# imkaywu/MVSKit

Hardware: AMD Instinct MI355X
Metric: patches/s (propagate+optim iteration), 12-view 1080p (higher is better)
Workload: dtype f32

## Files before the change

### include/mvskit_engine.h

```cpp
#ifndef MVSKIT_ENGINE_H
#define MVSKIT_ENGINE_H

#include <stddef.h>
#include <stdint.h>

#ifdef __cplusplus
extern "C" {
#endif

#ifndef MVS_MAX_IMAGES
#define MVS_MAX_IMAGES 32
#endif
#define MVS_LIST_CAP 16

typedef enum mvs_status {
    MVS_OK = 0,
    MVS_ERR_ARG = -1,
    MVS_ERR_STATE = -2,
    MVS_ERR_HIP = -3,
    MVS_ERR_CAPACITY = -4,
    MVS_ERR_NO_DEVICE = -5
} mvs_status;

typedef struct mvs_patch {
// ... 141 lines not shown
    MVS_PROBE_REFINE = 2,
    MVS_PROBE_POSTPROCESS = 3,
    MVS_PROBE_COST = 4,
    MVS_PROBE_MATH = 5,
    MVS_PROBE_REFINE_X = 6
} mvs_probe_op;
int mvs_engine_probe(mvs_engine* e, int op, int64_t n, const mvs_patch* in_rec, const float* in_f,
                     mvs_patch* out_rec, float* out_f, int32_t* out_i);

typedef struct mvs_timing {
    float index_ms;
    float sweep_ms;
    float commit_ms;
    int32_t sweep_launches;
    float exchange_ms;
    int64_t exchange_bytes;
    int64_t check_retried_cells;
} mvs_timing;
int mvs_engine_last_timing(mvs_engine* e, mvs_timing* t);

#ifdef __cplusplus
}
#endif
#endif
```

### mvskit_amd/csrc/mvs_engine.cpp

```cpp
#include <hip/hip_runtime.h>
#include <dlfcn.h>
#include <rccl/rccl.h>

#include <algorithm>
#include <climits>
#include <cmath>
#include <cstdio>
#include <cstdlib>
#include <cstring>
#include <string>
#include <vector>

#include "mvskit_engine.h"
#include "mvs_kernels.h"
#include "mvs_types.h"

static_assert(sizeof(mvs_patch) == sizeof(DPatch), "mvs_patch and DPatch must be the same bytes");
static_assert((MVS_LISTCAP == 16 || MVS_LISTCAP == 32 || MVS_LISTCAP == 64) && MVS_LISTCAP <= MVS_MAXI && MVS_MAX_IMAGES == MVS_MAXI, "limits out of sync");

namespace {
thread_local std::string g_err;

#define HIPCHK(expr)                                                                                       \
    do {                                                                                                   \
// ... 32 lines not shown
    }
    void release() { if (p) (void)hipFree(p); p = nullptr; cap = 0; }
};

namespace misc {
constexpr int stage_counter = 0;
constexpr int fill_evals = 1;
constexpr int neighbor_retry = 4;
constexpr int sweep_retry = 5;
constexpr int geo_bad = 6;
constexpr int group_edges = 7;
constexpr int trim_parts = 8;
constexpr int trim_nparts = 256;
constexpr int sweep_cursors = (trim_parts + trim_nparts + 15) / 16 * 16;
constexpr int sweep_cursor_words = MVS_SWEEP_QUEUES * MVS_SWEEP_CURSOR_STRIDE * (int)sizeof(uint32_t) / (int)sizeof(unsigned long long);
constexpr int words = sweep_cursors + sweep_cursor_words;
}
namespace fstat {
constexpr int neighbor_parts = 0;
constexpr int neighbor_cycles = 4096;
constexpr int exact_evals = 4112;
constexpr int words = exact_evals + 2048;
}

struct Rccl {
    void* h = nullptr;
    ncclResult_t (*GetUniqueId)(ncclUniqueId*) = nullptr;
    ncclResult_t (*CommInitRank)(ncclComm_t*, int, ncclUniqueId, int) = nullptr;
    ncclResult_t (*CommDestroy)(ncclComm_t) = nullptr;
    ncclResult_t (*CommCount)(const ncclComm_t, int*) = nullptr;
    ncclResult_t (*CommUserRank)(const ncclComm_t, int*) = nullptr;
// ... 90 lines not shown
    DevBuf<int32_t> group_edges;
    DevBuf<int32_t> cnt_alive, vcnt_alive;
    DevBuf<unsigned long long> dpgrid, best;
    DevBuf<uint32_t> dirty;
    bool dirty_marked = false;
    DevBuf<float4> geo;
    DevBuf<uint8_t> geo_ref;
    bool geo_valid = false;
    bool lists_dense[2] = {false, false};
    DevBuf<DPatch> staging;
    DevBuf<int32_t> job_stage, job_nstage, job_cnt, job_base_scan, kill_cnt, kill_base;
    DevBuf<unsigned long long> misc;
    DevBuf<DCounters> counters;
    DevBuf<int32_t> error_flag;
    DevBuf<int32_t> big_tables, retry_jobs;
    int64_t retried_cells = 0;
    int64_t pass_retried = 0;
    SweepArgs sa{};
    bool staged = false;
    bool counted = false;
    int64_t n_new = 0, n_kill = 0;
    std::vector<int32_t> h_per_view;
    DevBuf<DPatch> tmp_rec_in, tmp_rec_out;
    DevBuf<float> tmp_f_in, tmp_f_out;
    DevBuf<int32_t> tmp_i;
    DevBuf<uint8_t> tmp_bytes;
    hipEvent_t ev[6] = {nullptr, nullptr, nullptr, nullptr, nullptr, nullptr};
    mvs_timing timing{};
    mvs_filter_stats fstats{};
    int64_t fstats_exchange_bytes = 0;
// ... 586 lines not shown
        size_t free_b = 0, total_b = 0;
        if (hipMemGetInfo(&free_b, &total_b) == hipSuccess && total_b > 0) {
            pool_cap = std::max<int64_t>(std::min<int64_t>(pool_cap, (int64_t)(total_b / 6 / sizeof(DPatch))), std::min<int64_t>(pool_cap, nc));
            const double per_patch = 2.5 * (double)sizeof(DPatch) + 17.0;
            const int64_t fit = (int64_t)(0.6 * (double)free_b / per_patch);
            if (fit < pool_cap) pool_cap = std::max<int64_t>(fit, std::min<int64_t>(pool_cap, nc / 4 + 1024));
        }
    }
    e->ids.headroom = e->key.headroom = e->id32.headroom = e->id32_raw.headroom = e->vid32.headroom = true;
    e->geo.headroom = e->geo_ref.headroom = true;
    if (e->pool.ensure(pool_cap) || e->pool_alt.ensure(pool_cap) || e->kill.ensure(pool_cap) || e->kill_cnt.ensure(pool_cap + 2) || e->kill_base.ensure(pool_cap + 2)) return MVS_ERR_HIP;
    HIPCHK(hipMemsetAsync(e->kill.p, 0, (size_t)pool_cap, st));
    int64_t njobs_max = 0;
    for (int v = 0; v < nviews; ++v) njobs_max += (int64_t)((e->hviews[v].gw + 1) / 2) * e->hviews[v].gh;
    const int maxstage = (e->prm.view_propagation ? 3 : 2) * e->prm.cap * e->prm.max_propag;
    if (e->job_stage.ensure(njobs_max * maxstage) || e->job_nstage.ensure(njobs_max + 2) || e->job_cnt.ensure(njobs_max + 2) ||
        e->job_base_scan.ensure(njobs_max + 2))
        return MVS_ERR_HIP;
    const int64_t scan_n = std::max<int64_t>(std::max<int64_t>(nc, pool_cap), njobs_max);
    if (e->scan_tmp.ensure(scan_n / 256 + 4096)) return MVS_ERR_HIP;
    if (e->big_tables.ensure((int64_t)256 * 16384) || e->retry_jobs.ensure(std::max<int64_t>(njobs_max, 16))) return MVS_ERR_HIP;
    if (e->uf_parent.ensure(pool_cap) || e->uf_size.ensure(pool_cap) || e->dirty.ensure((nc + 31) / 32 + 1) || e->fstat_buf.ensure(fstat::words)) return MVS_ERR_HIP;
    if (e->staging.ensure(std::max<int64_t>(pool_cap / 2, 1024))) return MVS_ERR_HIP;
    if (e->tmp_rec_out.ensure(16)) return MVS_ERR_HIP;
    HIPCHK(hipStreamSynchronize(st));
    e->pool_n = 0;
    e->have_views = true;
    e->staged = false;
    return MVS_OK;
}

int mvs_engine_grid_dims(mvs_engine* e, int view, int* gw, int* gh) {
// ... 286 lines not shown
    if (e->kill.p && e->pool_n > 0) (void)hipMemsetAsync(e->kill.p, 0, (size_t)e->pool_n, e->stream);
    (void)hipStreamSynchronize(e->stream);
    e->staged = false; e->counted = false;
}
static int pass_impl(mvs_engine* e, int iter, int pass, mvs_counters* out) {
    if (!e || !e->have_views) { g_err = "mvs_engine_pass: views not set"; return MVS_ERR_STATE; }
    if (e->staged) { g_err = "mvs_engine_pass: the previous pass was not committed"; return MVS_ERR_STATE; }
    HIPCHK(hipSetDevice(e->cfg.device));
    hipStream_t st = e->stream;
    HIPCHK(hipEventRecord(e->ev[0], st));
    unsigned long long trimmed = 0;
    {
        Range rg("mvs:index");
        if (int r = build_index(e, &trimmed)) return r;
    }
    HIPCHK(hipEventRecord(e->ev[1], st));
    Range rg_sweep(pass & 1 ? "mvs:sweep colour 1" : "mvs:sweep colour 0");
    SweepArgs& a = e->sa;
    memset(&a, 0, sizeof a);
    a.iter = iter; a.inc = (iter % 2 == 0) ? 1 : -1; a.colour = pass & 1;
    int64_t nj = 0;
    const bool ranged = e->cfg.shard_count > 1;
    for (int v = ranged ? 0 : e->cfg.view_begin; v < e->cfg.nviews; v += ranged ? 1 : e->cfg.view_stride) {
        a.sweep_views[a.nsweep_views] = v;
        a.job_base[a.nsweep_views] = (int32_t)nj;
        ++a.nsweep_views;
        nj += (int64_t)((e->hviews[v].gw + 1) / 2) * e->hviews[v].gh;
    }
    a.njobs = nj;
    a.job_lo = 0; a.job_hi = nj;
    if (ranged) {
        const int split_mode = getenv("MVS_SPLIT_PROXY") ? atoi(getenv("MVS_SPLIT_PROXY")) : 2;
// ... 10 lines not shown
            HIPCHK(hipMemsetAsync(e->tmp_i.p, 0xff, (size_t)(N + 1) * sizeof(int32_t), st));
            mvsk_job_cuts(e->job_base_scan.p, nj, N, e->tmp_i.p, st);
            int32_t tw = 0;
            HIPCHK(hipMemcpyAsync(cuts.data(), e->tmp_i.p, (size_t)(N + 1) * sizeof(int32_t), hipMemcpyDeviceToHost, st));
            HIPCHK(hipMemcpyAsync(&tw, e->job_base_scan.p + nj, sizeof tw, hipMemcpyDeviceToHost, st));
            HIPCHK(hipStreamSynchronize(st));
            total_work = tw;
        }
        cuts[0] = 0; cuts[N] = (int32_t)nj;
        for (int r = 1; r < N; ++r) {
            if (total_work <= 0 || cuts[r] < 0) cuts[r] = (int32_t)(nj * r / N);
            cuts[r] = std::max(cuts[r], cuts[r - 1]);
        }
        a.job_lo = cuts[R];
        a.job_hi = cuts[R + 1];
        HIPCHK(hipMemsetAsync(e->job_nstage.p, 0, (size_t)nj * sizeof(int32_t), st));
    }
    a.staging = e->staging.p; a.staging_cap = e->staging.cap;
    a.stage_counter = e->misc.p + misc::stage_counter;
    a.job_stage = e->job_stage.p; a.job_nstage = e->job_nstage.p;
    a.maxstage = (e->prm.view_propagation ? 3 : 2) * e->prm.cap * e->prm.max_propag;
    a.kill = e->kill.p;
    a.counters = e->counters.p;
    a.error_flag = e->error_flag.p;
    if (want_vgrid(e)) {
        if (int r = e->big_tables.ensure((int64_t)256 * 16384)) return r;
        if (int r = e->retry_jobs.ensure(std::max<int64_t>(nj, 16))) return r;
    }
    a.big_tables = e->big_tables.p; a.retry_jobs = e->retry_jobs.p; a.nretry = reinterpret_cast<int32_t*>(e->misc.p + misc::sweep_retry);
    HIPCHK(hipMemsetAsync(e->misc.p + misc::sweep_retry, 0, sizeof(unsigned long long), st));
    HIPCHK(hipMemsetAsync(e->misc.p + misc::stage_counter, 0, sizeof(unsigned long long), st));
    a.cursors = reinterpret_cast<uint32_t*>(e->misc.p + misc::sweep_cursors);
    HIPCHK(hipMemsetAsync(e->misc.p + misc::sweep_cursors, 0, misc::sweep_cursor_words * sizeof(unsigned long long), st));
    HIPCHK(hipMemsetAsync(e->counters.p, 0, MVS_COUNTER_SLOTS * sizeof(DCounters), st));
    HIPCHK(hipMemsetAsync(e->error_flag.p, 0, sizeof(int32_t), st));
    const DParams p = current_params(e);
    const RefineSel rs = refine_sel(e);
    mvsk_sweep(p, a, rs, st);
    e->pass_retried = 0;
    if (want_vgrid(e)) {
        int32_t nretry = 0;
        HIPCHK(hipMemcpyAsync(&nretry, a.nretry, sizeof nretry, hipMemcpyDeviceToHost, st));
        HIPCHK(hipStreamSynchronize(st));
        e->pass_retried = nretry;
        if (nretry > 0) { mvsk_sweep_retry(p, a, nretry, rs, st); e->retried_cells += nretry; }
    }
    HIPCHK(hipEventRecord(e->ev[2], st));
    std::vector<DCounters> hcs(MVS_COUNTER_SLOTS);
    int32_t herr = 0;
    unsigned long long fill[2] = {0, 0};
    HIPCHK(hipMemcpyAsync(fill, e->misc.p + misc::fill_evals, sizeof fill, hipMemcpyDeviceToHost, st));
    HIPCHK(hipMemcpyAsync(hcs.data(), e->counters.p, hcs.size() * sizeof(DCounters), hipMemcpyDeviceToHost, st));
    HIPCHK(hipMemcpyAsync(&herr, e->error_flag.p, sizeof herr, hipMemcpyDeviceToHost, st));
    HIPCHK(hipStreamSynchronize(st));
    HIPCHK(hipGetLastError());
    mvs_counters sum{};
    for (const DCounters& c : hcs) add_counters(sum, c);
    sum.evals += fill[0]; sum.view_evals += fill[1]; sum.trimmed = (int64_t)trimmed;
    float ms = 0.0f;
    (void)hipEventElapsedTime(&ms, e->ev[0], e->ev[1]); e->timing.index_ms = ms;
    (void)hipEventElapsedTime(&ms, e->ev[1], e->ev[2]); e->timing.sweep_ms = ms;
    e->timing.commit_ms = 0.0f; e->timing.sweep_launches = 1; e->timing.exchange_ms = 0.0f; e->timing.exchange_bytes = 0;
    e->timing.check_retried_cells = e->pass_retried;
    e->staged = true; e->counted = false;
    if (out) *out = sum;
#ifdef MVS_STAGE_TIMING
    {
        unsigned long long stage[16] = {0};
        for (const DCounters& c : hcs)
            for (int k = 0; k < 16; ++k) stage[k] = (k == 12 || k == 13) ? std::max(stage[k], c.stage[k]) : stage[k] + c.stage[k];
        static const char* nm[8] = {"wave", "generate", "pre", "refine", "post", "check", "stage", "prologue"};
        fprintf(stderr, "[stage cycles]");
        for (int k = 0; k < 8; ++k) fprintf(stderr, " %s %.1f%%", nm[k], 100.0 * (double)stage[k] / (double)(stage[0] ? stage[0] : 1));
        static const char* nm2[4] = {"gain", "search", "sort", "quad"};
        for (int k = 0; k < 4; ++k) fprintf(stderr, " %s %.1f%%", nm2[k], 100.0 * (double)stage[8 + k] / (double)(stage[0] ? stage[0] : 1));
        fprintf(stderr, " setRefImage pairs %.1f%% choice %.1f%%", 100.0 * (double)stage[14] / (double)(stage[0] ? stage[0] : 1), 100.0 * (double)stage[15] / (double)(stage[0] ? stage[0] : 1));
        fprintf(stderr, "  (wave cycles %.3e; max visited %llu, max neighbours %llu)\n", (double)stage[0], stage[12], stage[13]);
    }
#endif
#ifdef MVS_FAULT_INJECTION
// ... 214 lines not shown
    memset(&total, 0, sizeof total);
    mvs_timing tt{};
    for (int pass = 0; pass < 2; ++pass) {
        mvs_counters c;
        memset(&c, 0, sizeof c);
        const int rp = mvs_engine_pass(e, iter, pass, &c);
        if (e && e->comm) {
            if (int r = mvs_engine_exchange(e)) return r;
        } else {
            if (rp) { if (e && e->staged) { const std::string keep = g_err; discard_pass(e); g_err = keep; } return rp; }
            if (int r = mvs_engine_commit_local(e)) return r;
        }
        add_counters(total, c);
        tt.index_ms += e->timing.index_ms; tt.sweep_ms += e->timing.sweep_ms; tt.commit_ms += e->timing.commit_ms; tt.sweep_launches += 1;
        tt.exchange_ms += e->timing.exchange_ms; tt.exchange_bytes += e->timing.exchange_bytes; tt.check_retried_cells += e->timing.check_retried_cells;
    }
    e->timing = tt;
    if (out) *out = total;
    return MVS_OK;
}

int mvs_engine_filter(mvs_engine* e, int64_t* removed4) {
    if (!e || !e->have_views) { g_err = "mvs_engine_filter: views not set"; return MVS_ERR_STATE; }
    if (e->staged) { g_err = "mvs_engine_filter: a pass is waiting for its commit"; return MVS_ERR_STATE; }
    HIPCHK(hipSetDevice(e->cfg.device));
    hipStream_t st = e->stream;
    int64_t rem[4] = {0, 0, 0, 0};
    Range rg("mvs:Filter::run");
    FilterRun fr{e};
    if (fr.multi()) { if (int r = e->comm_counts.ensure(MVS_XCHG_WORDS * (1 + (int64_t)e->comm_world))) return r; }
// ... 212 lines not shown
```

### mvskit_amd/csrc/mvs_kernels.h

```cpp
#pragma once
#include <hip/hip_runtime.h>
#include "mvs_types.h"

void mvsk_rgb_to_rgba(const uint8_t* rgb, uint32_t* out, int64_t n, hipStream_t st);
void mvsk_rgba_to_rgb(const uint32_t* in, uint8_t* rgb, int64_t n, hipStream_t st);
void mvsk_pyr_down(const uint32_t* src, int pw, int ph, uint32_t* dst, int w, int h, hipStream_t st);
void mvsk_mask_down(const uint8_t* src, int pw, int ph, uint8_t* dst, int w, int h, hipStream_t st);
void mvsk_mask_binarise(uint8_t* m, int64_t n, hipStream_t st);
void mvsk_exclusive_scan(const int32_t* in, int32_t* out, int64_t n, int32_t* tmp, hipStream_t st);
void mvsk_index_count(const DParams& prm, int32_t* cnt, int32_t* vcnt, unsigned long long* total, hipStream_t st);
void mvsk_exclusive_scan_off(const int32_t* in, csr_off_t* out, int64_t n, csr_off_t* tmp, hipStream_t st);
void mvsk_index_fill(const DParams& prm, int vgrid, const csr_off_t* start, int32_t* cursor, unsigned long long* ids, hipStream_t st);
void mvsk_index_fill_direct(const DParams& prm, int vgrid, const csr_off_t* start, int32_t* cursor, int32_t* id32, hipStream_t st);
void mvsk_index_sort_trim(const DParams& prm, const csr_off_t* start, unsigned long long* ids, int do_trim, unsigned long long* trimmed, hipStream_t st);
void mvsk_index_finalize(const DParams& prm, int vgrid, const csr_off_t* start, unsigned long long* ids, int32_t* id32, int32_t* cnt_alive, hipStream_t st);
void mvsk_index_pack(const DParams& prm, const csr_off_t* start, const csr_off_t* start2, const int32_t* cnt_alive, const unsigned long long* ids, const int32_t* id32_in,
                     ListKey* key, int32_t* id32_out, hipStream_t st);
void mvsk_depth_maps(const DParams& prm, unsigned long long* dp, const uint32_t* dirty, hipStream_t st);
void mvsk_depth_mark_dirty(const DParams& prm, const uint8_t* kill, unsigned long long* dp, uint32_t* dirty, hipStream_t st);
void mvsk_best_ncc_map(const DParams& prm, int view, unsigned long long* best, hipStream_t st);
void mvsk_map_extract(const DParams& prm, int view, int kind, const unsigned long long* sel, float* depth, float* normal, int32_t* ids, int ncells, hipStream_t st);
void mvsk_fill_ncc(const DParams& prm, unsigned long long* evals, hipStream_t st);
struct RefineSel { int simplex; int max_evals; float xtol; };
size_t mvsk_sweep_lds_bytes(const DParams& prm);
void mvsk_sweep(const DParams& prm, const SweepArgs& a, const RefineSel& rs, hipStream_t st);
void mvsk_sweep_retry(const DParams& prm, const SweepArgs& a, int nretry, const RefineSel& rs, hipStream_t st);
void mvsk_job_work(const DParams& prm, const SweepArgs& a, int mode, int shift, int32_t* work, hipStream_t st);
void mvsk_job_cuts(const int32_t* scan, int64_t njobs, int n, int32_t* cuts, hipStream_t st);
void mvsk_commit_count(const SweepArgs& a, int32_t* cnt, hipStream_t st);
void mvsk_commit_copy(const SweepArgs& a, const int32_t* base, DPatch* dst, int64_t dst_cap, int32_t* per_view, int keep_key, hipStream_t st);
void mvsk_kill_count(const uint8_t* kill, int64_t n, int32_t* cnt, hipStream_t st);
void mvsk_kill_export(const uint8_t* kill, int64_t n, const int32_t* base, int32_t* ids, int64_t cap, hipStream_t st);
void mvsk_apply_kill_flags(DPatch* pool, uint8_t* kill, int64_t n, hipStream_t st);
void mvsk_apply_kill_ids(DPatch* pool, const int32_t* ids, int64_t n, int64_t pool_n, hipStream_t st);
void mvsk_append_records(DPatch* pool, int64_t pool_n, const DPatch* recs, int64_t n, hipStream_t st);
void mvsk_alive_count(const DPatch* pool, int64_t n, int32_t* cnt, hipStream_t st);
void mvsk_alive_gather(const DPatch* pool, int64_t n, const int32_t* base, DPatch* out, int64_t cap, hipStream_t st);
void mvsk_filter_vimages(const DParams& prm, int additive, int64_t first, int64_t last, const uint32_t* dirty, hipStream_t st);
void mvsk_geo_pack(const DPatch* pool, int64_t n, float4* geo, uint8_t* ref, int* bad, hipStream_t st);
void mvsk_filter_outside(const DParams& prm, uint8_t* kill, int64_t first, int64_t last, hipStream_t st);
void mvsk_filter_exact(const DParams& prm, uint8_t* kill, unsigned long long* evals, unsigned long long* stage, int64_t first, int64_t last, hipStream_t st);
void mvsk_filter_neighbor(const DParams& prm, uint8_t* kill, int32_t* retry, int32_t* nretry, int32_t* overflow, unsigned long long* stats, int64_t first, int64_t last, hipStream_t st);
// ... 21 lines not shown
```

### mvskit_amd/csrc/mvs_kernels.hip

```cpp
#include <hip/hip_runtime.h>
#include <algorithm>
#include "mvs_device.cuh"
#include "mvs_check.cuh"
#include "mvs_kernels.h"

using namespace mvsdev;

__global__ void k_rgb_to_rgba(const uint8_t* __restrict__ rgb, uint32_t* __restrict__ out, int64_t n) {
    const int64_t i = (int64_t)blockIdx.x * blockDim.x + threadIdx.x;
    if (i >= n) return;
    const uint8_t* p = rgb + 3 * i;
    out[i] = (uint32_t)p[0] | ((uint32_t)p[1] << 8) | ((uint32_t)p[2] << 16);
}
__global__ void k_rgba_to_rgb(const uint32_t* __restrict__ in, uint8_t* __restrict__ rgb, int64_t n) {
    const int64_t i = (int64_t)blockIdx.x * blockDim.x + threadIdx.x;
    if (i >= n) return;
    const uint32_t t = in[i];
    rgb[3 * i] = t & 255u; rgb[3 * i + 1] = (t >> 8) & 255u; rgb[3 * i + 2] = (t >> 16) & 255u;
}
__global__ void k_pyr_down(const uint32_t* __restrict__ src, int pw, int ph, uint32_t* __restrict__ dst, int w, int h) {
    const int x = blockIdx.x * blockDim.x + threadIdx.x, y = blockIdx.y * blockDim.y + threadIdx.y;
    if (x >= w || y >= h) return;
    const float base[4] = {1.0f, 3.0f, 3.0f, 1.0f};
    float c0 = 0.0f, c1 = 0.0f, c2 = 0.0f;
// ... 293 lines not shown
        if (wc.lane == 0) p->ncc = ncc;
    }
    if (wc.lane == 0 && wc.evals) { atomicAdd(evals, (unsigned long long)wc.evals); atomicAdd(evals + 1, (unsigned long long)wc.view_evals); }
}

DEV bool rank_before(float na, int a, float nb, int b) { return (na != nb) ? (na > nb) : (a < b); }
DEV void job_cell(const DParams& prm, const SweepArgs& a, int64_t job, int& v, int& cx, int& cy) {
    int s = 0;
    while (s + 1 < a.nsweep_views && job >= a.job_base[s + 1]) ++s;
    v = a.sweep_views[s];
    const int gw = (prm.views + v)->gw, halfw = (gw + 1) / 2;
    const int local = (int)(job - a.job_base[s]);
    cy = local / halfw;
    cx = 2 * (local % halfw) + ((a.colour + cy) & 1);
}
DEV bool job_has_source(const DParams& prm, const SweepArgs& a, int64_t job) {
    int v, cx, cy;
    job_cell(prm, a, job, v, cx, cy);
    const DView* vw = prm.views + v;
    const int gw = vw->gw, gh = vw->gh;
    if (cx >= gw || cy >= gh) return false;
    const int sxs[2] = {cx, cx - a.inc}, sys[2] = {cy - a.inc, cy};
    bool has = false;
    for (int k = 0; k < 2; ++k) {
        if (sxs[k] < 0 || gw <= sxs[k] || sys[k] < 0 || gh <= sys[k]) continue;
        const int g = vw->cell_base + sys[k] * gw + sxs[k];
        has |= prm.csr_cnt[g] > 0;
    }
    if (prm.view_propagation) has |= prm.csr_cnt[vw->cell_base + cy * gw + cx] > 0;
    return has;
}
__global__ void k_job_work(DParams prm, SweepArgs a, int mode, int shift, int32_t* __restrict__ work) {
    const int64_t job = (int64_t)blockIdx.x * blockDim.x + threadIdx.x;
    if (job >= a.njobs) return;
    int v, cx, cy;
    job_cell(prm, a, job, v, cx, cy);
    const DView* vw = prm.views + v;
    const int gw = vw->gw, gh = vw->gh;
    int w = 0;
    if (cx < gw && cy < gh) {
        const int sxs[3] = {cx, cx - a.inc, cx}, sys[3] = {cy - a.inc, cy, cy};
        const int nsrc = prm.view_propagation ? 3 : 2;
        int n = 0;
        for (int k = 0; k < nsrc; ++k) {
            if (sxs[k] < 0 || gw <= sxs[k] || sys[k] < 0 || gh <= sys[k]) continue;
            const int g = vw->cell_base + sys[k] * gw + sxs[k];
            const csr_off_t sb = prm.csr_start[g];
            const int sn = prm.csr_cnt[g];
            for (int j = 0; j < sn; ++j) n += ((pgrid_ref(prm, sb + j) == v) != (k == 2)) ? 1 : 0;
        }
        if (mode == 1) w = n;
        else {
            const int trials = n * prm.max_propag;
            const int room = max(prm.cap - prm.csr_cnt[vw->cell_base + cy * gw + cx], 0);
            const int full = min(trials, (room * 5 + 3) / 4);
            w = 32 * full + 2 * (trials - full);
        }
    }
    work[job] = (w + (1 << shift) - 1) >> shift;
}
__global__ void k_job_cuts(const int32_t* __restrict__ scan, int64_t njobs, int n, int32_t* __restrict__ cuts) {
    const int64_t job = (int64_t)blockIdx.x * blockDim.x + threadIdx.x;
    if (job >= njobs) return;
    const long long total = scan[njobs], p0 = scan[job], p1 = scan[job + 1];
    if (p0 == p1) return;
    for (int r = 1; r < n; ++r) {
        const long long target = total * r / n;
        if (p0 <= target && target < p1) cuts[r] = (int32_t)job;
    }
}

#ifndef MVS_SWEEP_WAVES
#define MVS_SWEEP_WAVES 3
#endif
#ifdef MVS_STAGE_TIMING
#define ST_NOW() ((unsigned long long)__builtin_amdgcn_s_memtime())
#define ST_ADD(k, t0) { const unsigned long long t1_ = ST_NOW(); st_acc[k] += t1_ - (t0); (t0) = t1_; }
#else
#define ST_ADD(k, t0)
#endif
#ifndef MVS_XCD_CHUNK
#define MVS_XCD_CHUNK 128
#endif
struct SweepAcc {
    unsigned cand, pref, patch, f0, f1, ins, rep;
    unsigned long long evals, view_evals;
#ifdef MVS_STAGE_TIMING
    unsigned long long stage[16];
#endif
};
DEV SweepAcc sweep_acc_zero() {
    SweepAcc acc;
    acc.cand = acc.pref = acc.patch = acc.f0 = acc.f1 = acc.ins = acc.rep = 0u;
    acc.evals = acc.view_evals = 0ull;
#ifdef MVS_STAGE_TIMING
    for (int k = 0; k < 16; ++k) acc.stage[k] = 0ull;
#endif
// ... 157 lines not shown
        return;
    }
    if (wc.lane == 0) a.job_nstage[job] = ns;
    {
        acc->cand += n_cand; acc->pref += n_pref; acc->patch += n_patch; acc->f0 += n_f0; acc->f1 += n_f1; acc->ins += n_ins; acc->rep += n_rep;
        acc->evals += wc.evals; acc->view_evals += wc.view_evals;
#ifdef MVS_STAGE_TIMING
        st_acc[0] = ST_NOW() - st_begin;
        for (int k = 0; k < 12; ++k) acc->stage[k] += st_acc[k];
        acc->stage[12] = max(acc->stage[12], st_acc[12]); acc->stage[13] = max(acc->stage[13], st_acc[13]);
        acc->stage[14] += wc.st_acc[3]; acc->stage[15] += wc.st_acc[4];
#endif
    }
}

#ifndef MVS_SWEEP_TAKE
#define MVS_SWEEP_TAKE 1
#endif
static_assert(MVS_SWEEP_TAKE <= 64 && MVS_XCD_CHUNK % MVS_SWEEP_TAKE == 0, "a take is a part of one chunk, a lane per job");
template <bool SIMPLEX>
DEV void sweep_resident(const DParams& prm, const SweepArgs& a, int* s_scratch, float* s_texs, int max_evals, float xtol) {
    WaveCtx wc = make_wave_ctx(prm);
    SweepAcc acc = sweep_acc_zero();
    const int nchunks = (int)((a.job_hi - a.job_lo + MVS_XCD_CHUNK - 1) / MVS_XCD_CHUNK);
    constexpr unsigned per = MVS_XCD_CHUNK / MVS_SWEEP_TAKE;
    for (unsigned step = 0; step < MVS_SWEEP_QUEUES; ++step) {
        const unsigned q = (blockIdx.x + step) & (MVS_SWEEP_QUEUES - 1u);
        const unsigned ntake = (unsigned)((nchunks - (int)q + MVS_SWEEP_QUEUES - 1) / MVS_SWEEP_QUEUES) * per;
        for (;;) {
            unsigned k = 0;
            if (wc.lane == 0) k = atomicAdd(a.cursors + q * MVS_SWEEP_CURSOR_STRIDE, 1u);
            k = (unsigned)rfl((int)k);
            if (k >= ntake) break;
            const int64_t base = a.job_lo + ((int64_t)q + (int64_t)MVS_SWEEP_QUEUES * (k / per)) * MVS_XCD_CHUNK + (int64_t)(k % per) * MVS_SWEEP_TAKE;
            const int64_t mine = base + wc.lane;
            bool has = false;
            if (wc.lane < MVS_SWEEP_TAKE && mine < a.job_hi) {
                a.job_nstage[mine] = 0;
                has = job_has_source(prm, a, mine);
            }
            unsigned long long t = ballot(has);
            while (t) {
                const int l = __ffsll((long long)t) - 1;
                t &= t - 1ull;
                __syncthreads();
                sweep_cell<false, SIMPLEX>(prm, a, wc, &acc, base + l, s_scratch, s_texs, nullptr, max_evals, xtol);
            }
        }
    }
    if (wc.lane == 0) sweep_acc_flush(a, acc, blockIdx.x & (MVS_COUNTER_SLOTS - 1));
}
__global__ __launch_bounds__(64, MVS_SWEEP_WAVES) void k_sweep(DParams prm, SweepArgs a) {
    __shared__ int s_scratch[192];
    extern __shared__ float s_texs[];
    sweep_resident<false>(prm, a, s_scratch, s_texs, 0, 0.0f);
}
__global__ __launch_bounds__(64, MVS_SWEEP_WAVES) void k_sweep_simplex(DParams prm, SweepArgs a, int max_evals, float xtol) {
    __shared__ int s_scratch[192];
    extern __shared__ float s_texs[];
    sweep_resident<true>(prm, a, s_scratch, s_texs, max_evals, xtol);
}
template <bool SIMPLEX>
// ... 576 lines not shown
    const size_t texs = MVS_FRAME1_LDS_BYTES + (ln * 3 * prm.wsz + ln * (ln - 1) / 2) * sizeof(float);
#endif
    const size_t chk = (size_t)MVS_CHECK_LDS_FLOATS * sizeof(float);
    const size_t need = texs > chk ? texs : chk;
    return need > (size_t)MVS_FRAME_LDS_BYTES ? need : (size_t)MVS_FRAME_LDS_BYTES;
}
void mvsk_sweep(const DParams& prm, const SweepArgs& a, const RefineSel& rs, hipStream_t st) {
    const int64_t nloc = a.job_hi - a.job_lo;
    if (nloc <= 0) return;
    static const size_t pad = getenv("MVS_SWEEP_LDS_PAD") ? (size_t)atol(getenv("MVS_SWEEP_LDS_PAD")) : 0;
    const size_t lds = mvsk_sweep_lds_bytes(prm) + pad;
    int dev = 0, cus = 0;
    (void)hipGetDevice(&dev);
    if (hipDeviceGetAttribute(&cus, hipDeviceAttributeMultiprocessorCount, dev) != hipSuccess || cus <= 0) { (void)hipGetLastError(); cus = 256; }
    int64_t nblocks = (int64_t)cus * 4 * MVS_SWEEP_WAVES;
    nblocks = std::min(nblocks, (nloc + MVS_SWEEP_TAKE - 1) / MVS_SWEEP_TAKE);
    if (const char* g = getenv("MVS_SWEEP_GRID")) {
        const long cap = atol(g);
        if (cap > 0) nblocks = std::min<int64_t>(nblocks, cap);
    }
    if (rs.simplex) hipLaunchKernelGGL(k_sweep_simplex, dim3((unsigned)nblocks), dim3(64), lds, st, prm, a, rs.max_evals, rs.xtol);
    else hipLaunchKernelGGL(k_sweep, dim3((unsigned)nblocks), dim3(64), lds, st, prm, a);
}
void mvsk_job_work(const DParams& prm, const SweepArgs& a, int mode, int shift, int32_t* work, hipStream_t st) {
    if (a.njobs > 0) hipLaunchKernelGGL(k_job_work, dim3(nblk(a.njobs, 256)), dim3(256), 0, st, prm, a, mode, shift, work);
}
void mvsk_job_cuts(const int32_t* scan, int64_t njobs, int n, int32_t* cuts, hipStream_t st) {
    if (njobs > 0) hipLaunchKernelGGL(k_job_cuts, dim3(nblk(njobs, 256)), dim3(256), 0, st, scan, njobs, n, cuts);
}
void mvsk_sweep_retry(const DParams& prm, const SweepArgs& a, int nretry, const RefineSel& rs, hipStream_t st) {
    if (nretry <= 0) return;
    const dim3 grid((unsigned)std::min(nretry, MVS_BIG_SLOTS));
    if (rs.simplex) hipLaunchKernelGGL(k_sweep_retry_simplex, grid, dim3(64), mvsk_sweep_lds_bytes(prm), st, prm, a, nretry, rs.max_evals, rs.xtol);
    else hipLaunchKernelGGL(k_sweep_retry, grid, dim3(64), mvsk_sweep_lds_bytes(prm), st, prm, a, nretry);
}
void mvsk_commit_count(const SweepArgs& a, int32_t* cnt, hipStream_t st) { hipLaunchKernelGGL(k_commit_count, dim3(nblk(a.njobs, 256)), dim3(256), 0, st, a, cnt); }
void mvsk_commit_copy(const SweepArgs& a, const int32_t* base, DPatch* dst, int64_t dst_cap, int32_t* per_view, int keep_key, hipStream_t st) {
    hipLaunchKernelGGL(k_commit_copy, dim3(nblk(a.njobs, 256)), dim3(256), 0, st, a, base, dst, dst_cap, per_view, keep_key);
}
void mvsk_kill_count(const uint8_t* kill, int64_t n, int32_t* cnt, hipStream_t st) { if (n > 0) hipLaunchKernelGGL(k_kill_count, dim3(nblk(n, 256)), dim3(256), 0, st, kill, n, cnt); }
// ... 89 lines not shown
```

### mvskit_amd/csrc/mvs_types.h

```cpp
#pragma once
#include <stdint.h>

#define MVS_WAVE 64
#define MVS_MAXLEV 7
#ifndef MVS_LISTCAP
#define MVS_LISTCAP 16
#endif
#if MVS_LISTCAP > 32
#define MVS_MAXI 64
#else
#define MVS_MAXI 32
#endif
#define MVS_MAXVIEWS 64
#define MVS_CAPMAX 32
#define MVS_NEWBASE 0x40000000

#define MVS_FLAG_ALIVE 1
#define MVS_FLAG_SETTLED 2
struct DPatch {
    float coord[4];
    float normal[4];
    float ncc, dscale, ascale, tmp;
    int32_t nimages, nvimages, flags, id;
    uint8_t images[MVS_MAXI];
// ... 70 lines not shown
    int64_t njobs;
    int64_t job_lo, job_hi;
    DPatch* staging;
    int64_t staging_cap;
    unsigned long long* stage_counter;
    int32_t* job_stage;
    int32_t* job_nstage;
    int32_t maxstage;
    uint8_t* kill;
    DCounters* counters;
    int32_t* error_flag;
    int32_t* big_tables;
    int32_t* retry_jobs;
    int32_t* nretry;
    uint32_t* cursors;
};
```

### mvskit_amd/engine.py

```python
from __future__ import annotations

import ctypes as C
import os

import numpy as np

from . import build
from . import synth
from .synth import MAX_IMAGES, PATCH_DTYPE

PROBE_NCC, PROBE_PREPROCESS, PROBE_REFINE, PROBE_POSTPROCESS, PROBE_COST, PROBE_MATH, PROBE_REFINE_X = range(7)
REFINE_HALVING, REFINE_CONVERGED = 0, 1

EXPORTS = [
    "mvs_last_error", "mvs_device_count", "mvs_default_config", "mvs_engine_create", "mvs_engine_destroy",
    "mvs_engine_set_views", "mvs_engine_grid_dims", "mvs_engine_get_pyramid", "mvs_engine_set_thresholds",
    "mvs_engine_get_thresholds", "mvs_engine_update_threshold", "mvs_engine_upload_patches",
    "mvs_engine_clear_patches", "mvs_engine_num_patches", "mvs_engine_download_patches", "mvs_engine_propagate",
    "mvs_engine_pass", "mvs_engine_export_counts", "mvs_engine_export_device", "mvs_engine_commit_device",
    "mvs_engine_commit_local", "mvs_engine_depth_normal_map", "mvs_engine_probe", "mvs_engine_last_timing",
    "mvs_engine_filter", "mvs_comm_unique_id", "mvs_engine_comm_init", "mvs_engine_comm_attach", "mvs_engine_comm_release",
    "mvs_engine_exchange", "mvs_list_cap", "mvs_engine_filter_stats", "mvs_patch_bytes", "mvs_engine_reserve", "mvs_engine_comm_info",
    "mvs_default_refiner", "mvs_engine_set_refiner", "mvs_engine_export_ply", "mvs_engine_seed_patches",
]
# ... 22 lines not shown

class SeedView(C.Structure):
    _fields_ = [("normals", C.c_void_p), ("mask", C.c_void_p)]


class Counters(C.Structure):
    _fields_ = [(n, C.c_int64) for n in ("candidates", "prefiltered", "patches", "fail0", "fail1", "inserted",
                                         "replaced", "evals", "view_evals", "trimmed")]

    def as_dict(self):
        return {n: int(getattr(self, n)) for n, _ in self._fields_}


class Timing(C.Structure):
    _fields_ = [("index_ms", C.c_float), ("sweep_ms", C.c_float), ("commit_ms", C.c_float), ("sweep_launches", C.c_int32),
                ("exchange_ms", C.c_float), ("exchange_bytes", C.c_int64), ("check_retried_cells", C.c_int64)]


class FilterStats(C.Structure):
    _fields_ = [(n, C.c_float) for n in ("outside_ms", "exact_ms", "neighbor_ms", "groups_ms", "rebuild_ms", "total_ms")] + \
               [(n, C.c_int64) for n in ("patches_in", "exact_patches", "exact_view_evals", "neighbor_patches", "neighbor_tasks", "neighbor_entries",
                                         "neighbor_visited", "neighbor_accepted", "neighbor_retried", "exchange_bytes")]


class EngineError(RuntimeError):

    def __init__(self, msg, status=None):
        super().__init__(msg)
        self.status = status


# ... 265 lines not shown
        r, w, cc, cr = C.c_int(), C.c_int(), C.c_int(), C.c_int()
        self.L.mvs_engine_comm_info.argtypes = [C.c_void_p] + [C.POINTER(C.c_int)] * 4
        self._check(self.L.mvs_engine_comm_info(self.h, C.byref(r), C.byref(w), C.byref(cc), C.byref(cr)))
        return {"rank": r.value, "world": w.value, "comm_count": cc.value, "comm_rank": cr.value}

    def comm_release(self):
        self._check(self.L.mvs_engine_comm_release(self.h))

    def exchange(self):
        self._check(self.L.mvs_engine_exchange(self.h))

    def timing(self):
        t = Timing()
        self._check(self.L.mvs_engine_last_timing(self.h, C.byref(t)))
        return {"index_ms": t.index_ms, "sweep_ms": t.sweep_ms, "commit_ms": t.commit_ms, "sweep_launches": t.sweep_launches,
                "exchange_ms": t.exchange_ms, "exchange_bytes": int(t.exchange_bytes), "check_retried_cells": int(t.check_retried_cells)}

    def depth_normal_map(self, view, kind):
        gw, gh = self.grid_dims(view)
        d = np.zeros((gh, gw), np.float32)
        n = np.zeros((gh, gw, 3), np.float32)
        ids = np.zeros((gh, gw), np.int32)
        self._check(self.L.mvs_engine_depth_normal_map(self.h, view, kind, _ptr(d), _ptr(n), _ptr(ids)))
        return d, n, ids

    def probe(self, op, recs=None, values=None):
        if op == PROBE_MATH:
            x = np.ascontiguousarray(values, dtype=np.float32)
            out = np.zeros((x.shape[0], 5), np.float32)
            self._check(self.L.mvs_engine_probe(self.h, op, x.shape[0], None, _ptr(x), None, _ptr(out), None))
            return out
# ... 8 lines not shown
```

Measured before the change: 28.90 million.

## Compact sweep jobs into per-queue lists before the resident sweep kernel

Adds a pre-pass that flags each job with at least one same-view trial source, scans the flags and scatters the surviving job ids into a compacted list with per-queue bounds. The resident sweep kernel then pulls jobs straight from this list instead of claiming 128-job chunks and ballot-checking each lane for a source. The source test is now stricter, counting matching-view entries rather than any non-empty neighbour cell, so fewer empty jobs should reach the heavy sweep. The cost is three extra launches plus a scan per pass, and the job_nstage reset moves into the list kernel.

```diff
diff --git a/include/mvskit_engine.h b/include/mvskit_engine.h
--- a/include/mvskit_engine.h
+++ b/include/mvskit_engine.h
@@ -179,6 +179,7 @@
     float commit_ms;
     int32_t sweep_launches;
     float exchange_ms;
+    int32_t sweep_jobs_listed;
     int64_t exchange_bytes;
     int64_t check_retried_cells;
 } mvs_timing;
diff --git a/mvskit_amd/csrc/mvs_engine.cpp b/mvskit_amd/csrc/mvs_engine.cpp
--- a/mvskit_amd/csrc/mvs_engine.cpp
+++ b/mvskit_amd/csrc/mvs_engine.cpp
@@ -70,7 +70,10 @@
 constexpr int trim_nparts = 256;
 constexpr int sweep_cursors = (trim_parts + trim_nparts + 15) / 16 * 16;
 constexpr int sweep_cursor_words = MVS_SWEEP_QUEUES * MVS_SWEEP_CURSOR_STRIDE * (int)sizeof(uint32_t) / (int)sizeof(unsigned long long);
-constexpr int words = sweep_cursors + sweep_cursor_words;
+constexpr int sweep_list_bounds = sweep_cursors + sweep_cursor_words;
+constexpr int sweep_list_bound_words = (MVS_SWEEP_QUEUES + 1 + 1) / 2;
+constexpr int words = sweep_list_bounds + sweep_list_bound_words;
+constexpr int64_t job_list_pad = 1024 + 2;
 }
 namespace fstat {
 constexpr int neighbor_parts = 0;
@@ -191,6 +194,7 @@
     DevBuf<DCounters> counters;
     DevBuf<int32_t> error_flag;
     DevBuf<int32_t> big_tables, retry_jobs;
+    DevBuf<int32_t> job_list;
     int64_t retried_cells = 0;
     int64_t pass_retried = 0;
     SweepArgs sa{};
@@ -807,8 +811,8 @@
     int64_t njobs_max = 0;
     for (int v = 0; v < nviews; ++v) njobs_max += (int64_t)((e->hviews[v].gw + 1) / 2) * e->hviews[v].gh;
     const int maxstage = (e->prm.view_propagation ? 3 : 2) * e->prm.cap * e->prm.max_propag;
-    if (e->job_stage.ensure(njobs_max * maxstage) || e->job_nstage.ensure(njobs_max + 2) || e->job_cnt.ensure(njobs_max + 2) ||
-        e->job_base_scan.ensure(njobs_max + 2))
+    if (e->job_stage.ensure(njobs_max * maxstage) || e->job_nstage.ensure(njobs_max + 2) || e->job_cnt.ensure(njobs_max + misc::job_list_pad) ||
+        e->job_base_scan.ensure(njobs_max + misc::job_list_pad) || e->job_list.ensure(std::max<int64_t>(njobs_max, 16)))
         return MVS_ERR_HIP;
     const int64_t scan_n = std::max<int64_t>(std::max<int64_t>(nc, pool_cap), njobs_max);
     if (e->scan_tmp.ensure(scan_n / 256 + 4096)) return MVS_ERR_HIP;
@@ -1125,8 +1129,6 @@
         Range rg("mvs:index");
         if (int r = build_index(e, &trimmed)) return r;
     }
-    HIPCHK(hipEventRecord(e->ev[1], st));
-    Range rg_sweep(pass & 1 ? "mvs:sweep colour 1" : "mvs:sweep colour 0");
     SweepArgs& a = e->sa;
     memset(&a, 0, sizeof a);
     a.iter = iter; a.inc = (iter % 2 == 0) ? 1 : -1; a.colour = pass & 1;
@@ -1167,7 +1169,6 @@
         }
         a.job_lo = cuts[R];
         a.job_hi = cuts[R + 1];
-        HIPCHK(hipMemsetAsync(e->job_nstage.p, 0, (size_t)nj * sizeof(int32_t), st));
     }
     a.staging = e->staging.p; a.staging_cap = e->staging.cap;
     a.stage_counter = e->misc.p + misc::stage_counter;
@@ -1184,11 +1185,18 @@
     HIPCHK(hipMemsetAsync(e->misc.p + misc::sweep_retry, 0, sizeof(unsigned long long), st));
     HIPCHK(hipMemsetAsync(e->misc.p + misc::stage_counter, 0, sizeof(unsigned long long), st));
     a.cursors = reinterpret_cast<uint32_t*>(e->misc.p + misc::sweep_cursors);
-    HIPCHK(hipMemsetAsync(e->misc.p + misc::sweep_cursors, 0, misc::sweep_cursor_words * sizeof(unsigned long long), st));
+    HIPCHK(hipMemsetAsync(e->misc.p + misc::sweep_cursors, 0, (misc::sweep_cursor_words + misc::sweep_list_bound_words) * sizeof(unsigned long long), st));
     HIPCHK(hipMemsetAsync(e->counters.p, 0, MVS_COUNTER_SLOTS * sizeof(DCounters), st));
     HIPCHK(hipMemsetAsync(e->error_flag.p, 0, sizeof(int32_t), st));
     const DParams p = current_params(e);
     const RefineSel rs = refine_sel(e);
+    if (int r = e->job_list.ensure(std::max<int64_t>(nj, 16))) return r;
+    if (e->job_cnt.ensure(nj + misc::job_list_pad) || e->job_base_scan.ensure(nj + misc::job_list_pad)) return MVS_ERR_HIP;
+    int32_t* list_bounds = reinterpret_cast<int32_t*>(e->misc.p + misc::sweep_list_bounds);
+    a.job_list = e->job_list.p; a.list_bounds = list_bounds;
+    mvsk_job_list(p, a, e->job_cnt.p, e->job_base_scan.p, reinterpret_cast<int32_t*>(e->scan_tmp.p), e->job_list.p, list_bounds, st);
+    HIPCHK(hipEventRecord(e->ev[1], st));
+    Range rg_sweep(pass & 1 ? "mvs:sweep colour 1" : "mvs:sweep colour 0");
     mvsk_sweep(p, a, rs, st);
     e->pass_retried = 0;
     if (want_vgrid(e)) {
@@ -1205,6 +1213,8 @@
     HIPCHK(hipMemcpyAsync(fill, e->misc.p + misc::fill_evals, sizeof fill, hipMemcpyDeviceToHost, st));
     HIPCHK(hipMemcpyAsync(hcs.data(), e->counters.p, hcs.size() * sizeof(DCounters), hipMemcpyDeviceToHost, st));
     HIPCHK(hipMemcpyAsync(&herr, e->error_flag.p, sizeof herr, hipMemcpyDeviceToHost, st));
+    int32_t hbounds[MVS_SWEEP_QUEUES + 1];
+    HIPCHK(hipMemcpyAsync(hbounds, list_bounds, sizeof hbounds, hipMemcpyDeviceToHost, st));
     HIPCHK(hipStreamSynchronize(st));
     HIPCHK(hipGetLastError());
     mvs_counters sum{};
@@ -1215,8 +1225,13 @@
     (void)hipEventElapsedTime(&ms, e->ev[1], e->ev[2]); e->timing.sweep_ms = ms;
     e->timing.commit_ms = 0.0f; e->timing.sweep_launches = 1; e->timing.exchange_ms = 0.0f; e->timing.exchange_bytes = 0;
     e->timing.check_retried_cells = e->pass_retried;
+    e->timing.sweep_jobs_listed = hbounds[MVS_SWEEP_QUEUES];
     e->staged = true; e->counted = false;
     if (out) *out = sum;
+#ifdef MVS_JOBLIST_COUNTS
+    fprintf(stderr, "[job list] iter %d colour %d: jobs %lld, with any source entry %llu, listed %llu\n", iter, pass & 1, (long long)(a.job_hi - a.job_lo),
+            hcs[0].stage[0], hcs[0].stage[1]);
+#endif
 #ifdef MVS_STAGE_TIMING
     {
         unsigned long long stage[16] = {0};
@@ -1461,6 +1476,7 @@
         add_counters(total, c);
         tt.index_ms += e->timing.index_ms; tt.sweep_ms += e->timing.sweep_ms; tt.commit_ms += e->timing.commit_ms; tt.sweep_launches += 1;
         tt.exchange_ms += e->timing.exchange_ms; tt.exchange_bytes += e->timing.exchange_bytes; tt.check_retried_cells += e->timing.check_retried_cells;
+        tt.sweep_jobs_listed += e->timing.sweep_jobs_listed;
     }
     e->timing = tt;
     if (out) *out = total;
diff --git a/mvskit_amd/csrc/mvs_kernels.h b/mvskit_amd/csrc/mvs_kernels.h
--- a/mvskit_amd/csrc/mvs_kernels.h
+++ b/mvskit_amd/csrc/mvs_kernels.h
@@ -26,6 +26,8 @@
 void mvsk_sweep(const DParams& prm, const SweepArgs& a, const RefineSel& rs, hipStream_t st);
 void mvsk_sweep_retry(const DParams& prm, const SweepArgs& a, int nretry, const RefineSel& rs, hipStream_t st);
 void mvsk_job_work(const DParams& prm, const SweepArgs& a, int mode, int shift, int32_t* work, hipStream_t st);
+int mvsk_job_list_seg(const SweepArgs& a);
+void mvsk_job_list(const DParams& prm, const SweepArgs& a, int32_t* flags, int32_t* scan, int32_t* scan_tmp, int32_t* list, int32_t* bounds, hipStream_t st);
 void mvsk_job_cuts(const int32_t* scan, int64_t njobs, int n, int32_t* cuts, hipStream_t st);
 void mvsk_commit_count(const SweepArgs& a, int32_t* cnt, hipStream_t st);
 void mvsk_commit_copy(const SweepArgs& a, const int32_t* base, DPatch* dst, int64_t dst_cap, int32_t* per_view, int keep_key, hipStream_t st);
diff --git a/mvskit_amd/csrc/mvs_kernels.hip b/mvskit_amd/csrc/mvs_kernels.hip
--- a/mvskit_amd/csrc/mvs_kernels.hip
+++ b/mvskit_amd/csrc/mvs_kernels.hip
@@ -331,45 +331,37 @@
     cy = local / halfw;
     cx = 2 * (local % halfw) + ((a.colour + cy) & 1);
 }
-DEV bool job_has_source(const DParams& prm, const SweepArgs& a, int64_t job) {
+DEV int job_trial_sources(const DParams& prm, const SweepArgs& a, int64_t job, int* dest) {
     int v, cx, cy;
     job_cell(prm, a, job, v, cx, cy);
     const DView* vw = prm.views + v;
     const int gw = vw->gw, gh = vw->gh;
-    if (cx >= gw || cy >= gh) return false;
-    const int sxs[2] = {cx, cx - a.inc}, sys[2] = {cy - a.inc, cy};
-    bool has = false;
-    for (int k = 0; k < 2; ++k) {
+    *dest = -1;
+    if (cx >= gw || cy >= gh) return 0;
+    *dest = vw->cell_base + cy * gw + cx;
+    const int sxs[3] = {cx, cx - a.inc, cx}, sys[3] = {cy - a.inc, cy, cy};
+    const int nsrc = prm.view_propagation ? 3 : 2;
+    int n = 0;
+    for (int k = 0; k < nsrc; ++k) {
         if (sxs[k] < 0 || gw <= sxs[k] || sys[k] < 0 || gh <= sys[k]) continue;
         const int g = vw->cell_base + sys[k] * gw + sxs[k];
-        has |= prm.csr_cnt[g] > 0;
-    }
-    if (prm.view_propagation) has |= prm.csr_cnt[vw->cell_base + cy * gw + cx] > 0;
-    return has;
+        const csr_off_t sb = prm.csr_start[g];
+        const int sn = min(prm.csr_cnt[g], MVS_CAPMAX);
+        for (int j = 0; j < sn; ++j) n += ((pgrid_ref(prm, sb + j) == v) != (k == 2)) ? 1 : 0;
+    }
+    return n;
 }
 __global__ void k_job_work(DParams prm, SweepArgs a, int mode, int shift, int32_t* __restrict__ work) {
     const int64_t job = (int64_t)blockIdx.x * blockDim.x + threadIdx.x;
     if (job >= a.njobs) return;
-    int v, cx, cy;
-    job_cell(prm, a, job, v, cx, cy);
-    const DView* vw = prm.views + v;
-    const int gw = vw->gw, gh = vw->gh;
+    int dest;
+    const int n = job_trial_sources(prm, a, job, &dest);
     int w = 0;
-    if (cx < gw && cy < gh) {
-        const int sxs[3] = {cx, cx - a.inc, cx}, sys[3] = {cy - a.inc, cy, cy};
-        const int nsrc = prm.view_propagation ? 3 : 2;
-        int n = 0;
-        for (int k = 0; k < nsrc; ++k) {
-            if (sxs[k] < 0 || gw <= sxs[k] || sys[k] < 0 || gh <= sys[k]) continue;
-            const int g = vw->cell_base + sys[k] * gw + sxs[k];
-            const csr_off_t sb = prm.csr_start[g];
-            const int sn = prm.csr_cnt[g];
-            for (int j = 0; j < sn; ++j) n += ((pgrid_ref(prm, sb + j) == v) != (k == 2)) ? 1 : 0;
-        }
+    if (dest >= 0) {
         if (mode == 1) w = n;
         else {
             const int trials = n * prm.max_propag;
-            const int room = max(prm.cap - prm.csr_cnt[vw->cell_base + cy * gw + cx], 0);
+            const int room = max(prm.cap - prm.csr_cnt[dest], 0);
             const int full = min(trials, (room * 5 + 3) / 4);
             w = 32 * full + 2 * (trials - full);
         }
@@ -387,6 +379,48 @@
     }
 }
 
+#ifndef MVS_XCD_CHUNK
+#define MVS_XCD_CHUNK 128
+#endif
+DEV int64_t list_slot_job(const SweepArgs& a, int64_t slot, int seg) {
+    const int64_t q = slot / seg, r = slot % seg;
+    return a.job_lo + ((r / MVS_XCD_CHUNK) * MVS_SWEEP_QUEUES + q) * MVS_XCD_CHUNK + r % MVS_XCD_CHUNK;
+}
+__global__ void k_job_list(DParams prm, SweepArgs a, int seg, int32_t* __restrict__ flags) {
+    const int64_t t = (int64_t)blockIdx.x * blockDim.x + threadIdx.x;
+    if (t < a.njobs) a.job_nstage[t] = 0;
+    if (t >= (int64_t)MVS_SWEEP_QUEUES * seg) return;
+    const int64_t job = list_slot_job(a, t, seg);
+    int dest = -1;
+    const int n = job < a.job_hi ? job_trial_sources(prm, a, job, &dest) : 0;
+    flags[t] = n > 0 ? 1 : 0;
+#ifdef MVS_JOBLIST_COUNTS
+    bool any = false;
+    if (dest >= 0) {
+        int v, cx, cy;
+        job_cell(prm, a, job, v, cx, cy);
+        const DView* vw = prm.views + v;
+        const int sxs[3] = {cx, cx - a.inc, cx}, sys[3] = {cy - a.inc, cy, cy};
+        for (int k = 0; k < (prm.view_propagation ? 3 : 2); ++k)
+            if (0 <= sxs[k] && sxs[k] < vw->gw && 0 <= sys[k] && sys[k] < vw->gh) any |= prm.csr_cnt[vw->cell_base + sys[k] * vw->gw + sxs[k]] > 0;
+    }
+    const unsigned long long m_any = __ballot(any), m_listed = __ballot(n > 0);
+    if ((threadIdx.x & 63) == 0) {
+        if (m_any) atomicAdd(&a.counters->stage[0], (unsigned long long)__popcll(m_any));
+        if (m_listed) atomicAdd(&a.counters->stage[1], (unsigned long long)__popcll(m_listed));
+    }
+#endif
+}
+__global__ void k_job_scatter(SweepArgs a, int seg, const int32_t* __restrict__ scan, int32_t* __restrict__ list, int32_t* __restrict__ bounds) {
+    const int64_t t = (int64_t)blockIdx.x * blockDim.x + threadIdx.x;
+    const int64_t nslots = (int64_t)MVS_SWEEP_QUEUES * seg;
+    if (t >= nslots) return;
+    const int32_t pos = scan[t];
+    if (t % seg == 0) bounds[t / seg] = pos;
+    if (t == nslots - 1) bounds[MVS_SWEEP_QUEUES] = scan[nslots];
+    if (scan[t + 1] != pos) list[pos] = (int32_t)list_slot_job(a, t, seg);
+}
+
 #ifndef MVS_SWEEP_WAVES
 #define MVS_SWEEP_WAVES 3
 #endif
@@ -395,9 +429,6 @@
 #define ST_ADD(k, t0) { const unsigned long long t1_ = ST_NOW(); st_acc[k] += t1_ - (t0); (t0) = t1_; }
 #else
 #define ST_ADD(k, t0)
-#endif
-#ifndef MVS_XCD_CHUNK
-#define MVS_XCD_CHUNK 128
 #endif
 struct SweepAcc {
     unsigned cand, pref, patch, f0, f1, ins, rep;
@@ -585,38 +616,23 @@
     }
 }
 
-#ifndef MVS_SWEEP_TAKE
-#define MVS_SWEEP_TAKE 1
-#endif
-static_assert(MVS_SWEEP_TAKE <= 64 && MVS_XCD_CHUNK % MVS_SWEEP_TAKE == 0, "a take is a part of one chunk, a lane per job");
 template <bool SIMPLEX>
 DEV void sweep_resident(const DParams& prm, const SweepArgs& a, int* s_scratch, float* s_texs, int max_evals, float xtol) {
     WaveCtx wc = make_wave_ctx(prm);
     SweepAcc acc = sweep_acc_zero();
-    const int nchunks = (int)((a.job_hi - a.job_lo + MVS_XCD_CHUNK - 1) / MVS_XCD_CHUNK);
-    constexpr unsigned per = MVS_XCD_CHUNK / MVS_SWEEP_TAKE;
     for (unsigned step = 0; step < MVS_SWEEP_QUEUES; ++step) {
         const unsigned q = (blockIdx.x + step) & (MVS_SWEEP_QUEUES - 1u);
-        const unsigned ntake = (unsigned)((nchunks - (int)q + MVS_SWEEP_QUEUES - 1) / MVS_SWEEP_QUEUES) * per;
+        const int32_t qbegin = a.list_bounds[q];
+        const unsigned ntake = (unsigned)(a.list_bounds[q + 1] - qbegin);
+        if (ntake == 0u) continue;
         for (;;) {
             unsigned k = 0;
             if (wc.lane == 0) k = atomicAdd(a.cursors + q * MVS_SWEEP_CURSOR_STRIDE, 1u);
             k = (unsigned)rfl((int)k);
             if (k >= ntake) break;
-            const int64_t base = a.job_lo + ((int64_t)q + (int64_t)MVS_SWEEP_QUEUES * (k / per)) * MVS_XCD_CHUNK + (int64_t)(k % per) * MVS_SWEEP_TAKE;
-            const int64_t mine = base + wc.lane;
-            bool has = false;
-            if (wc.lane < MVS_SWEEP_TAKE && mine < a.job_hi) {
-                a.job_nstage[mine] = 0;
-                has = job_has_source(prm, a, mine);
-            }
-            unsigned long long t = ballot(has);
-            while (t) {
-                const int l = __ffsll((long long)t) - 1;
-                t &= t - 1ull;
-                __syncthreads();
-                sweep_cell<false, SIMPLEX>(prm, a, wc, &acc, base + l, s_scratch, s_texs, nullptr, max_evals, xtol);
-            }
+            const int64_t job = a.job_list[qbegin + (int32_t)k];
+            __syncthreads();
+            sweep_cell<false, SIMPLEX>(prm, a, wc, &acc, job, s_scratch, s_texs, nullptr, max_evals, xtol);
         }
     }
     if (wc.lane == 0) sweep_acc_flush(a, acc, blockIdx.x & (MVS_COUNTER_SLOTS - 1));
@@ -1223,7 +1239,7 @@
     (void)hipGetDevice(&dev);
     if (hipDeviceGetAttribute(&cus, hipDeviceAttributeMultiprocessorCount, dev) != hipSuccess || cus <= 0) { (void)hipGetLastError(); cus = 256; }
     int64_t nblocks = (int64_t)cus * 4 * MVS_SWEEP_WAVES;
-    nblocks = std::min(nblocks, (nloc + MVS_SWEEP_TAKE - 1) / MVS_SWEEP_TAKE);
+    nblocks = std::min(nblocks, nloc);
     if (const char* g = getenv("MVS_SWEEP_GRID")) {
         const long cap = atol(g);
         if (cap > 0) nblocks = std::min<int64_t>(nblocks, cap);
@@ -1233,6 +1249,19 @@
 }
 void mvsk_job_work(const DParams& prm, const SweepArgs& a, int mode, int shift, int32_t* work, hipStream_t st) {
     if (a.njobs > 0) hipLaunchKernelGGL(k_job_work, dim3(nblk(a.njobs, 256)), dim3(256), 0, st, prm, a, mode, shift, work);
+}
+int mvsk_job_list_seg(const SweepArgs& a) {
+    const int64_t nchunks = (std::max<int64_t>(a.job_hi - a.job_lo, 0) + MVS_XCD_CHUNK - 1) / MVS_XCD_CHUNK;
+    return (int)((nchunks + MVS_SWEEP_QUEUES - 1) / MVS_SWEEP_QUEUES) * MVS_XCD_CHUNK;
+}
+void mvsk_job_list(const DParams& prm, const SweepArgs& a, int32_t* flags, int32_t* scan, int32_t* scan_tmp, int32_t* list, int32_t* bounds, hipStream_t st) {
+    const int seg = mvsk_job_list_seg(a);
+    const int64_t nslots = (int64_t)MVS_SWEEP_QUEUES * seg, nthreads = std::max(nslots, a.njobs);
+    if (nthreads <= 0) return;
+    hipLaunchKernelGGL(k_job_list, dim3(nblk(nthreads, 256)), dim3(256), 0, st, prm, a, seg, flags);
+    if (nslots <= 0) return;
+    launch_exclusive_scan<int32_t, int32_t>(flags, scan, nslots, scan_tmp, st);
+    hipLaunchKernelGGL(k_job_scatter, dim3(nblk(nslots, 256)), dim3(256), 0, st, a, seg, scan, list, bounds);
 }
 void mvsk_job_cuts(const int32_t* scan, int64_t njobs, int n, int32_t* cuts, hipStream_t st) {
     if (njobs > 0) hipLaunchKernelGGL(k_job_cuts, dim3(nblk(njobs, 256)), dim3(256), 0, st, scan, njobs, n, cuts);
diff --git a/mvskit_amd/csrc/mvs_types.h b/mvskit_amd/csrc/mvs_types.h
--- a/mvskit_amd/csrc/mvs_types.h
+++ b/mvskit_amd/csrc/mvs_types.h
@@ -108,4 +108,6 @@
     int32_t* retry_jobs;
     int32_t* nretry;
     uint32_t* cursors;
+    const int32_t* job_list;
+    const int32_t* list_bounds;
 };
diff --git a/mvskit_amd/engine.py b/mvskit_amd/engine.py
--- a/mvskit_amd/engine.py
+++ b/mvskit_amd/engine.py
@@ -60,7 +60,7 @@
 
 class Timing(C.Structure):
     _fields_ = [("index_ms", C.c_float), ("sweep_ms", C.c_float), ("commit_ms", C.c_float), ("sweep_launches", C.c_int32),
-                ("exchange_ms", C.c_float), ("exchange_bytes", C.c_int64), ("check_retried_cells", C.c_int64)]
+                ("exchange_ms", C.c_float), ("sweep_jobs_listed", C.c_int32), ("exchange_bytes", C.c_int64), ("check_retried_cells", C.c_int64)]
 
 
 class FilterStats(C.Structure):
@@ -356,7 +356,8 @@
         t = Timing()
         self._check(self.L.mvs_engine_last_timing(self.h, C.byref(t)))
         return {"index_ms": t.index_ms, "sweep_ms": t.sweep_ms, "commit_ms": t.commit_ms, "sweep_launches": t.sweep_launches,
-                "exchange_ms": t.exchange_ms, "exchange_bytes": int(t.exchange_bytes), "check_retried_cells": int(t.check_retried_cells)}
+                "exchange_ms": t.exchange_ms, "exchange_bytes": int(t.exchange_bytes), "check_retried_cells": int(t.check_retried_cells),
+                "sweep_jobs_listed": int(t.sweep_jobs_listed)}
 
     def depth_normal_map(self, view, kind):
         gw, gh = self.grid_dims(view)
```

Result: faster. 29.92 million (median of 6 runs) (+3.6%).
